# CPJKU/beat_this

Measured on NVIDIA H100. Metric: clips/sec (30 s audio->beats, final0), higher is better.
Workload: dtype f16

## Files before the change

beat_this_b200/csrc/kernels_attn.cu:

```cuda
#include <cstdio>

#include "tc_common.cuh"

namespace bt {

constexpr int AT_BQ = 128;
constexpr int AT_BKV = 64;
constexpr int AT_NST = 4;
constexpr int AT_WARPS = 8;
constexpr int AT_THREADS = 32 * (AT_WARPS + 1);
constexpr int AT_SQ = AT_BQ * 64;
constexpr int AT_SKV = AT_BKV * 64;
constexpr int AT_SMEM = 1024 + AT_SQ + AT_NST * 2 * AT_SKV + 128;

constexpr uint32_t AT_POLY_MASK = 0x52u;

__device__ __forceinline__ uint32_t sw64_off(int r, int c) {
  return static_cast<uint32_t>(r * 64 + ((c ^ ((r >> 1) & 3)) << 4));
}

__global__ void __launch_bounds__(AT_THREADS, 2)
attn_time_kernel(const __grid_constant__ CUtensorMap tmQ, const __grid_constant__ CUtensorMap tmKV,
                 const float* __restrict__ gates, h16* __restrict__ out, int L, int heads,
                 const ChunkSrc* __restrict__ chunks, int seqs_per_chunk) {
  extern __shared__ uint8_t smem_raw[];
  const uint32_t sbase = (smem_u32(smem_raw) + 1023u) & ~1023u;
  const uint32_t sQ = sbase;
  const uint32_t sK = sQ + AT_SQ;
  const uint32_t sV = sK + AT_NST * AT_SKV;
  const uint32_t bar_q = sV + AT_NST * AT_SKV;
  const uint32_t full = bar_q + 8;
  const uint32_t empty = full + 8 * AT_NST;

  const int warp = threadIdx.x >> 5, lane = threadIdx.x & 31;
  const int q0 = blockIdx.x * AT_BQ;
  const int h = blockIdx.y;
  const int seq = blockIdx.z;
  const int C = heads * 32;
  const int Lk = chunks ? chunks[seq / seqs_per_chunk].len : L;
  const int nkv = ceil_div(Lk, AT_BKV);

  if (threadIdx.x == 0) {
    mbar_init(bar_q, 1);
    for (int i = 0; i < AT_NST; ++i) {
      mbar_init(full + 8 * i, 1);
      mbar_init(empty + 8 * i, AT_WARPS);
    }
    fence_barrier_init();
  }
  __syncthreads();

  if (warp == AT_WARPS) {
    if (lane == 0) {
      tma_prefetch_desc(&tmQ);
      tma_prefetch_desc(&tmKV);
      mbar_expect_tx(bar_q, AT_SQ);
      tma_load_3d(sQ, &tmQ, bar_q, h * 32, q0, seq);
      for (int j = 0; j < nkv; ++j) {
        const int st = j % AT_NST;
        if (j >= AT_NST) mbar_wait(empty + 8 * st, ((j / AT_NST) - 1) & 1);
        mbar_expect_tx(full + 8 * st, 2 * AT_SKV);
        tma_load_3d(sK + st * AT_SKV, &tmKV, full + 8 * st, C + h * 32, j * AT_BKV, seq);
        tma_load_3d(sV + st * AT_SKV, &tmKV, full + 8 * st, 2 * C + h * 32, j * AT_BKV, seq);
      }
    }
    return;
  }

  const int r0 = warp * 16;
  mbar_wait(bar_q, 0);
  uint32_t qa[2][4];
#pragma unroll
  for (int ks = 0; ks < 2; ++ks) ldmatrix_x4(sQ + sw64_off(r0 + (lane & 15), 2 * ks + (lane >> 4)), qa[ks]);

  float o[4][4];
#pragma unroll
  for (int d = 0; d < 4; ++d) o[d][0] = o[d][1] = o[d][2] = o[d][3] = 0.f;
  float m_run[2] = {-INFINITY, -INFINITY}, l_run[2] = {0.f, 0.f};
  for (int j = 0; j < nkv; ++j) {
    const int st = j % AT_NST;
    mbar_wait(full + 8 * st, (j / AT_NST) & 1);
    const uint32_t kb = sK + st * AT_SKV, vb = sV + st * AT_SKV;
    float s[8][4];
#pragma unroll
    for (int nb = 0; nb < 8; ++nb) {
      s[nb][0] = s[nb][1] = s[nb][2] = s[nb][3] = 0.f;
      uint32_t kf[4];
      ldmatrix_x4(kb + sw64_off(nb * 8 + (lane & 7), lane >> 3), kf);
      mma_16816(s[nb], qa[0], kf[0], kf[1]);
      mma_16816(s[nb], qa[1], kf[2], kf[3]);
    }
    if (j == nkv - 1) {
      const int lim = Lk - j * AT_BKV;
#pragma unroll
      for (int nb = 0; nb < 8; ++nb) {
        const int key = nb * 8 + 2 * (lane & 3);
        if (key >= lim) s[nb][0] = s[nb][2] = -INFINITY;
        if (key + 1 >= lim) s[nb][1] = s[nb][3] = -INFINITY;
      }
    }
    float mx[2] = {-INFINITY, -INFINITY};
#pragma unroll
    for (int nb = 0; nb < 8; ++nb) {
      mx[0] = fmaxf(mx[0], fmaxf(s[nb][0], s[nb][1]));
      mx[1] = fmaxf(mx[1], fmaxf(s[nb][2], s[nb][3]));
    }
    float mref[2], alpha[2];
#pragma unroll
    for (int r = 0; r < 2; ++r) {
      mx[r] = fmaxf(mx[r], __shfl_xor_sync(0xffffffffu, mx[r], 1));
      mx[r] = fmaxf(mx[r], __shfl_xor_sync(0xffffffffu, mx[r], 2));
      mref[r] = fmaxf(m_run[r], mx[r]);
      alpha[r] = ex2_approx(m_run[r] - mref[r]);
      m_run[r] = mref[r];
      l_run[r] *= alpha[r];
    }
#pragma unroll
    for (int d = 0; d < 4; ++d) {
      o[d][0] *= alpha[0]; o[d][1] *= alpha[0];
      o[d][2] *= alpha[1]; o[d][3] *= alpha[1];
    }
    uint32_t pa[4][4];
#pragma unroll
    for (int nb = 0; nb < 8; ++nb) {
      float p[4];
#pragma unroll
      for (int i = 0; i < 4; ++i) {
        const float x = s[nb][i] - mref[i >> 1];
        p[i] = ((AT_POLY_MASK >> nb) & 1u) ? ex2_poly(x) : ex2_approx(x);
      }
      l_run[0] += p[0] + p[1];
      l_run[1] += p[2] + p[3];
      pa[nb >> 1][(nb & 1) * 2] = pack_h16x2(p[0], p[1]);
      pa[nb >> 1][(nb & 1) * 2 + 1] = pack_h16x2(p[2], p[3]);
    }
#pragma unroll
    for (int kk = 0; kk < 4; ++kk) {
      const int key = kk * 16 + (lane & 7) + ((lane >> 3) & 1) * 8;
#pragma unroll
      for (int dp = 0; dp < 2; ++dp) {
        uint32_t vf[4];
        ldmatrix_x4_trans(vb + sw64_off(key, 2 * dp + (lane >> 4)), vf);
        mma_16816(o[2 * dp], pa[kk], vf[0], vf[1]);
        mma_16816(o[2 * dp + 1], pa[kk], vf[2], vf[3]);
      }
    }
    __syncwarp();
    if (lane == 0) mbar_arrive(empty + 8 * st);
  }
#pragma unroll
  for (int r = 0; r < 2; ++r) {
    l_run[r] += __shfl_xor_sync(0xffffffffu, l_run[r], 1);
    l_run[r] += __shfl_xor_sync(0xffffffffu, l_run[r], 2);
  }
#pragma unroll
  for (int r = 0; r < 2; ++r) {
    const int q = q0 + r0 + (lane >> 2) + 8 * r;
    if (q < L) {
      const int64_t m = static_cast<int64_t>(seq) * L + q;
      const float gsc = gates[m * heads + h] / l_run[r];
      h16* dst = out + m * C + h * 32 + 2 * (lane & 3);
#pragma unroll
      for (int d = 0; d < 4; ++d)
        *reinterpret_cast<uint32_t*>(dst + 8 * d) = pack_h16x2(o[d][2 * r] * gsc, o[d][2 * r + 1] * gsc);
    }
  }
}

struct TcAttnPlan {
  CUtensorMap tmQ;
  CUtensorMap tmKV;
  int seqs, L, heads;
};

TcAttnPlan* tc_attn_plan_create(const void* qkv, int seqs, int L, int heads, char* err, int errlen) {
  TcAttnPlan* p = new TcAttnPlan();
  p->seqs = seqs; p->L = L; p->heads = heads;
  const int C = heads * 32;
  const uint64_t dims[3] = {static_cast<uint64_t>(3 * C), static_cast<uint64_t>(L), static_cast<uint64_t>(seqs)};
  const uint64_t strides[2] = {static_cast<uint64_t>(3 * C) * 2, static_cast<uint64_t>(L) * 3 * C * 2};
  const uint32_t box_q[3] = {32, AT_BQ, 1};
  const uint32_t box_kv[3] = {32, AT_BKV, 1};
  if (!make_tmap(&p->tmQ, qkv, 3, dims, strides, box_q, 64, err, errlen) ||
      !make_tmap(&p->tmKV, qkv, 3, dims, strides, box_kv, 64, err, errlen)) {
    delete p;
    return nullptr;
  }
  return p;
}
void tc_attn_plan_destroy(TcAttnPlan* p) { delete p; }

void launch_attn_time_tc(const TcAttnPlan* p, const float* gates, void* out, cudaStream_t st, const ChunkSrc* chunks,
                         int seqs_per_chunk) {
  dim3 grid(ceil_div(p->L, AT_BQ), p->heads, p->seqs);
  attn_time_kernel<<<grid, AT_THREADS, AT_SMEM, st>>>(p->tmQ, p->tmKV, gates, reinterpret_cast<h16*>(out), p->L, p->heads,
                                                      chunks, seqs_per_chunk);
}

int tc_init_attn(char* err, int errlen) {
  const cudaError_t r = cudaFuncSetAttribute(attn_time_kernel, cudaFuncAttributeMaxDynamicSharedMemorySize, AT_SMEM);
  if (r != cudaSuccess) {
    snprintf(err, errlen, "cudaFuncSetAttribute(attn_time_kernel) failed: %s", cudaGetErrorString(r));
    return -1;
  }
  return 0;
}

}
```

Before: 750.6.

## Drop dedicated TMA producer warp, issue loads from consumer thread; precompute swizzle offsets

Removes the separate producer warp. Thread 0 of the consumer warps now issues the initial K/V prefetch and, inside the main loop, refills the slot freed in the previous iteration. It also precomputes the swizzled ldmatrix offsets as per-lane constants plus immediate strides, and skips the output rescale when every alpha in the warp is one. This saves one warp per CTA and some address arithmetic. The cost is that warp 0 stalls on the empty barrier before it can refill, which can delay the producer and serialize warp 0 behind the slowest warp.

```diff
diff --git a/beat_this_b200/csrc/kernels_attn.cu b/beat_this_b200/csrc/kernels_attn.cu
--- a/beat_this_b200/csrc/kernels_attn.cu
+++ b/beat_this_b200/csrc/kernels_attn.cu
@@ -4,11 +4,12 @@
 
 namespace bt {
 
-constexpr int AT_BQ = 128;
+constexpr int AT_WARPS = 8;
+constexpr int AT_CTAS_PER_SM = 2;
+constexpr int AT_BQ = 16 * AT_WARPS;
 constexpr int AT_BKV = 64;
 constexpr int AT_NST = 4;
-constexpr int AT_WARPS = 8;
-constexpr int AT_THREADS = 32 * (AT_WARPS + 1);
+constexpr int AT_THREADS = 32 * AT_WARPS;
 constexpr int AT_SQ = AT_BQ * 64;
 constexpr int AT_SKV = AT_BKV * 64;
 constexpr int AT_SMEM = 1024 + AT_SQ + AT_NST * 2 * AT_SKV + 128;
@@ -19,7 +20,7 @@
   return static_cast<uint32_t>(r * 64 + ((c ^ ((r >> 1) & 3)) << 4));
 }
 
-__global__ void __launch_bounds__(AT_THREADS, 2)
+__global__ void __launch_bounds__(AT_THREADS, AT_CTAS_PER_SM)
 attn_time_kernel(const __grid_constant__ CUtensorMap tmQ, const __grid_constant__ CUtensorMap tmKV,
                  const float* __restrict__ gates, h16* __restrict__ out, int L, int heads,
                  const ChunkSrc* __restrict__ chunks, int seqs_per_chunk) {
@@ -50,21 +51,18 @@
   }
   __syncthreads();
 
-  if (warp == AT_WARPS) {
-    if (lane == 0) {
-      tma_prefetch_desc(&tmQ);
-      tma_prefetch_desc(&tmKV);
-      mbar_expect_tx(bar_q, AT_SQ);
-      tma_load_3d(sQ, &tmQ, bar_q, h * 32, q0, seq);
-      for (int j = 0; j < nkv; ++j) {
-        const int st = j % AT_NST;
-        if (j >= AT_NST) mbar_wait(empty + 8 * st, ((j / AT_NST) - 1) & 1);
-        mbar_expect_tx(full + 8 * st, 2 * AT_SKV);
-        tma_load_3d(sK + st * AT_SKV, &tmKV, full + 8 * st, C + h * 32, j * AT_BKV, seq);
-        tma_load_3d(sV + st * AT_SKV, &tmKV, full + 8 * st, 2 * C + h * 32, j * AT_BKV, seq);
-      }
-    }
-    return;
+  auto load_kv = [&](int j) {
+    const int st = j % AT_NST;
+    mbar_expect_tx(full + 8 * st, 2 * AT_SKV);
+    tma_load_3d(sK + st * AT_SKV, &tmKV, full + 8 * st, C + h * 32, j * AT_BKV, seq);
+    tma_load_3d(sV + st * AT_SKV, &tmKV, full + 8 * st, 2 * C + h * 32, j * AT_BKV, seq);
+  };
+  if (threadIdx.x == 0) {
+    tma_prefetch_desc(&tmQ);
+    tma_prefetch_desc(&tmKV);
+    mbar_expect_tx(bar_q, AT_SQ);
+    tma_load_3d(sQ, &tmQ, bar_q, h * 32, q0, seq);
+    for (int j = 0; j < AT_NST && j < nkv; ++j) load_kv(j);
   }
 
   const int r0 = warp * 16;
@@ -72,6 +70,10 @@
   uint32_t qa[2][4];
 #pragma unroll
   for (int ks = 0; ks < 2; ++ks) ldmatrix_x4(sQ + sw64_off(r0 + (lane & 15), 2 * ks + (lane >> 4)), qa[ks]);
+
+  const uint32_t k_off = sw64_off(lane & 7, lane >> 3);
+  const uint32_t v_off = sw64_off((lane & 7) + ((lane >> 3) & 1) * 8, lane >> 4);
+  const uint32_t v_off1 = v_off ^ 32u;
 
   float o[4][4];
 #pragma unroll
@@ -79,14 +81,19 @@
   float m_run[2] = {-INFINITY, -INFINITY}, l_run[2] = {0.f, 0.f};
   for (int j = 0; j < nkv; ++j) {
     const int st = j % AT_NST;
+    if (threadIdx.x == 0 && j >= 1 && j + AT_NST - 1 < nkv) {
+      mbar_wait(empty + 8 * ((j - 1) % AT_NST), ((j - 1) / AT_NST) & 1);
+      load_kv(j + AT_NST - 1);
+    }
     mbar_wait(full + 8 * st, (j / AT_NST) & 1);
-    const uint32_t kb = sK + st * AT_SKV, vb = sV + st * AT_SKV;
+    const uint32_t kb = sK + st * AT_SKV + k_off;
+    const uint32_t vb0 = sV + st * AT_SKV + v_off, vb1 = sV + st * AT_SKV + v_off1;
     float s[8][4];
 #pragma unroll
     for (int nb = 0; nb < 8; ++nb) {
       s[nb][0] = s[nb][1] = s[nb][2] = s[nb][3] = 0.f;
       uint32_t kf[4];
-      ldmatrix_x4(kb + sw64_off(nb * 8 + (lane & 7), lane >> 3), kf);
+      ldmatrix_x4(kb + nb * 512, kf);
       mma_16816(s[nb], qa[0], kf[0], kf[1]);
       mma_16816(s[nb], qa[1], kf[2], kf[3]);
     }
@@ -99,9 +106,9 @@
         if (key + 1 >= lim) s[nb][1] = s[nb][3] = -INFINITY;
       }
     }
-    float mx[2] = {-INFINITY, -INFINITY};
-#pragma unroll
-    for (int nb = 0; nb < 8; ++nb) {
+    float mx[2] = {fmaxf(s[0][0], s[0][1]), fmaxf(s[0][2], s[0][3])};
+#pragma unroll
+    for (int nb = 1; nb < 8; ++nb) {
       mx[0] = fmaxf(mx[0], fmaxf(s[nb][0], s[nb][1]));
       mx[1] = fmaxf(mx[1], fmaxf(s[nb][2], s[nb][3]));
     }
@@ -115,6 +122,7 @@
       m_run[r] = mref[r];
       l_run[r] *= alpha[r];
     }
+    if (__any_sync(0xffffffffu, alpha[0] != 1.f || alpha[1] != 1.f))
 #pragma unroll
     for (int d = 0; d < 4; ++d) {
       o[d][0] *= alpha[0]; o[d][1] *= alpha[0];
@@ -136,11 +144,10 @@
     }
 #pragma unroll
     for (int kk = 0; kk < 4; ++kk) {
-      const int key = kk * 16 + (lane & 7) + ((lane >> 3) & 1) * 8;
 #pragma unroll
       for (int dp = 0; dp < 2; ++dp) {
         uint32_t vf[4];
-        ldmatrix_x4_trans(vb + sw64_off(key, 2 * dp + (lane >> 4)), vf);
+        ldmatrix_x4_trans((dp ? vb1 : vb0) + kk * 1024, vf);
         mma_16816(o[2 * dp], pa[kk], vf[0], vf[1]);
         mma_16816(o[2 * dp + 1], pa[kk], vf[2], vf[3]);
       }
```

Result: faster. 766.2, median of 6 (+2.1%).
